# arnauqb/GradABM-JUNE

Measured on AMD Instinct MI355X. Metric: simulation steps/sec, higher is better.
Workload: dtype f32

## Files before the change

### gradabm-june_amd/csrc/gj_compile.hip

```cpp
#include <hip/hip_runtime.h>
#include <hipcub/hipcub.hpp>
#include <stdint.h>

#include <algorithm>

#include "../../include/gradjune_hip.h"

namespace gjc {

constexpr int kThreads = 256;
constexpr int kPad = 8;
constexpr int kChunk = 64;
constexpr int kWideSegments = 6;

static inline int grid_for(int64_t n) { return (int)std::max<int64_t>(1, std::min<int64_t>((n + kThreads - 1) / kThreads, 1 << 18)); }
static inline int grid_for_reduction(int64_t n) { return (int)std::max<int64_t>(1, std::min<int64_t>((n + kThreads - 1) / kThreads, 2048)); }
static inline int64_t align_up(int64_t x) { return (x + 255) & ~(int64_t)255; }
static inline int bits_for(uint64_t n) {
  int b = 0;
  while (b < 64 && (n > ((uint64_t)1 << b))) ++b;
  return std::max(b, 1);
}

__device__ __forceinline__ int upper_bound(const int32_t* a, int n, int64_t x) {
// ... 213 lines not shown
}

__global__ void k_ell_fill(const uint32_t* keys, const uint32_t* order, int64_t E, int64_t n_agents,
                           const int32_t* rowptr, const int64_t* venue, int64_t rows, int32_t ell_k, uint16_t* ell,
                           int32_t* counts) {
  for (int64_t i = (int64_t)blockIdx.x * blockDim.x + threadIdx.x; i < E; i += (int64_t)gridDim.x * blockDim.x) {
    const uint32_t a = keys[i];
    if ((int64_t)a >= n_agents) continue;
    const int col = (int)i - rowptr[a];
    if (col < 0 || col >= ell_k) {
      if (counts) counts[GJ_CC_ERROR] = 5;
      continue;
    }
    ell[((int64_t)(col >> 1) * rows + a) * 2 + (col & 1)] = (uint16_t)venue[order[i]];
  }
}

__global__ void k_explicit_slots(const int32_t* sptr, const int32_t* tile_jpos, int64_t n_tiles, int64_t E, int32_t* slots) {
  for (int64_t i = (int64_t)blockIdx.x * blockDim.x + threadIdx.x; i < E; i += (int64_t)gridDim.x * blockDim.x) {
    int64_t lo = 0, hi = n_tiles + 1;
    while (lo < hi) {
      const int64_t mid = (lo + hi) >> 1;
      if ((int64_t)sptr[mid] > i) {
        hi = mid;
      } else {
        lo = mid + 1;
      }
    }
    const int64_t t = lo - 1;
    slots[i] = tile_jpos[t] + (int32_t)(i - sptr[t]);
// ... 430 lines not shown
  const int64_t need = 2 * gjc::align_up(n1 * 4) + gjc::align_up((int64_t)temp_bytes);
  if (need > workspace_bytes) return GJ_E_RANGE;
  char* base = static_cast<char*>(workspace);
  int32_t* flags = reinterpret_cast<int32_t*>(base);
  int32_t* rows = reinterpret_cast<int32_t*>(base + gjc::align_up(n1 * 4));
  void* temp = base + 2 * gjc::align_up(n1 * 4);
  hipStream_t st = (hipStream_t)stream;
  gjc::k_multi_flags<<<gjc::grid_for(n1), gjc::kThreads, 0, st>>>(desc, n_chunks, wide, flags);
  if (const int rc = gjc::exclusive_scan(temp, temp_bytes, flags, rows, n1, st)) return rc;
  gjc::k_multi_fill<<<gjc::grid_for((int64_t)n_chunks * 64), gjc::kThreads, 0, st>>>(
      out->chunk_ptr, out->tile_sptr, out->tile_jpos, set->n_blocks, set->n_slices, n_chunks, wide, rows, desc, multi_slots,
      counts);
  return (int)hipGetLastError();
}

int gj_compile_runs_pick(const gj_compile_set* set, int32_t* vmin, int32_t* pick, uint8_t* keep, int32_t* win_lo,
                         int32_t* win_n, int32_t* counts, void* stream) {
  if (const int rc = gjc::check_set(set)) return rc;
  if (!vmin || !pick || !counts || !win_lo || !win_n || (set->n_edges > 0 && !keep)) return GJ_E_NULL;
  if (set->n_venues >= gjc::kNoVenue) return GJ_E_RANGE;
  hipStream_t st = (hipStream_t)stream;
  const int64_t A = set->n_agents, E = set->n_edges;
  const int32_t n_own_slices = (int32_t)std::max<int64_t>(1, (A + set->slice_agents - 1) / set->slice_agents);
  GJC_HIP(hipMemsetAsync(counts, 0, GJ_COMPILE_COUNTS * sizeof(int32_t), st));
  if (A > 0) {
    GJC_HIP(hipMemsetD32Async((hipDeviceptr_t)vmin, gjc::kNoVenue, (size_t)A, st));
    GJC_HIP(hipMemsetD32Async((hipDeviceptr_t)pick, gjc::kNoVenue, (size_t)A, st));
  }
  if (E > 0 && A > 0) {
    gjc::k_run_vmin<<<gjc::grid_for(E), gjc::kThreads, 0, st>>>(set->agent, set->venue, E, A, vmin);
// ... 42 lines not shown
```

### gradabm-june_amd/csrc/gj_tiled.h

```cpp
#pragma once
#include <hip/hip_runtime.h>
#include <stdint.h>

#include <type_traits>

#include "../../include/gradjune_hip.h"
#include "gj_device.h"

namespace gj {

constexpr int kTileThreads = 1024;
constexpr int kTileWaves = kTileThreads / kWave;
constexpr int kMaxSliceAgents = 19840;
constexpr int kUnroll = 8;
#ifndef GJ_UNROLL_NARROW
#define GJ_UNROLL_NARROW 16
#endif
constexpr int kUnrollNarrow = GJ_UNROLL_NARROW;
#ifndef GJ_VENUE_UNROLL
#define GJ_VENUE_UNROLL 2
#endif
constexpr int kVenueUnroll = GJ_VENUE_UNROLL;
#ifndef GJ_VENUE_UNROLL_C
#define GJ_VENUE_UNROLL_C GJ_VENUE_UNROLL
// ... 416 lines not shown
      if (T.wide == 2) {
        scatter_explicit<kUnroll>(T, lds_x, s, wave, lane);
      } else if (T.wide) {
        scatter_set<true>(T, lds_x, s, wave, lane);
      } else {
        scatter_set<false>(T, lds_x, s, wave, lane);
      }
    }
  }
}

struct TSetB {
  const int32_t* blk_v0;
  const int32_t* blk_e0;
  const uint16_t* e_lv;
  const uint8_t* e_cls;
  float* val;
  const float* v_pc;
  float* cum;
  int32_t stride;
  int32_t nk;
  float beta[GJ_MAX_NETS_PER_SET];
  int32_t table[GJ_MAX_NETS_PER_SET];
  int32_t age75[GJ_MAX_NETS_PER_SET];
  int32_t leisure;
  int32_t direct;
  uint32_t term_limit;
  int32_t multinet;
  const uint16_t* pv_blk;
  const int32_t* blk_r0;
// ... 61 lines not shown
      : w{raw.x, raw.y, raw.z, raw.w}, c{craw.x, craw.y}, v{xa.x, xa.y, xa.z, xa.w, xb.x, xb.y, xb.z, xb.w} {}
  __device__ __forceinline__ int lv(int q) const { return (w[q >> 1] >> ((q & 1) * 16)) & 0xFFFF; }
  __device__ __forceinline__ float x(int q) const { return v[q]; }
  __device__ __forceinline__ int cls(int q) const { return class_byte(c[q >> 2], q & 3); }
  __device__ __forceinline__ void drop(int q) { w[q >> 1] |= 0xFFFFu << ((q & 1) * 16); }
  __device__ __forceinline__ bool one_venue() const {
    return (w[0] == w[1]) && (w[1] == w[2]) && (w[2] == w[3]) && ((w[0] >> 16) == (w[0] & 0xFFFFu)) && (lv(0) != 0xFFFF);
  }
  __device__ __forceinline__ Group8 weighted(const float* tk) const {
    Group8 g = *this;
#pragma unroll
    for (int q = 0; q < 8; ++q) g.v[q] = tk[cls(q)] * v[q];
    return g;
  }
};

#ifdef GJ_DIAG_STAMPS
constexpr int kDiagVenueSlots = 8192;
__device__ unsigned long long gj_diag_venue[3 * kDiagVenueSlots];
struct VenueStamp {
  unsigned long long t0;
  __device__ VenueStamp() : t0(__builtin_amdgcn_s_memrealtime()) {}
  __device__ ~VenueStamp() {
    if (threadIdx.x == 0 && blockIdx.x < kDiagVenueSlots) {
      gj_diag_venue[3 * blockIdx.x] = t0;
      gj_diag_venue[3 * blockIdx.x + 1] = __builtin_amdgcn_s_memrealtime();
      gj_diag_venue[3 * blockIdx.x + 2] = __builtin_amdgcn_s_getreg((31 << 11) | 20) & 0xF;
    }
  }
};
// ... 8 lines not shown
  int g0, g1;
  fx_t* sums;
  float* cumf;
  int wpad;
  float* tabs;
  float* tabs2;
  uint32_t* vflags;
  int vwords;
  int dummy;
  __device__ __forceinline__ VenueItem(const TSetB& T_, int j, float* lds, int tid_)
      : T(T_), tid(tid_), nk(T_.nk), v0(T_.blk_v0[j]), nv(T_.blk_v0[j + 1] - v0), g0(T_.blk_e0[j] >> 3),
        g1(T_.blk_e0[j + 1] >> 3), sums(reinterpret_cast<fx_t*>(lds)), cumf(lds), wpad(T_.multinet ? class_pad(nk) : 0),
        tabs(lds + 2 * (((size_t)nk * nv + 64 + 1) & ~(size_t)1)), tabs2(tabs + (T_.leisure ? (wpad ? wpad : nk) * 200 : 0)),
        vflags(reinterpret_cast<uint32_t*>(tabs2 + (T_.leisure ? nk * 200 : 0))), vwords((nk * nv + 64 + 31) / 32),
        dummy(nk * nv + (tid_ & 63)) {}
  __device__ __forceinline__ const uint4* lv8() const { return reinterpret_cast<const uint4*>(T.e_lv); }
  __device__ __forceinline__ const uint2* cls8() const { return reinterpret_cast<const uint2*>(T.e_cls); }
  __device__ __forceinline__ float4* val4() const { return reinterpret_cast<float4*>(T.val); }
};

__device__ __forceinline__ void run_sums(const VenueItem& W, const Group8& G, int base_k, fx_t* sums, uint32_t* vflags) {
  const uint32_t kLimit = W.T.term_limit;
  static_assert(kFxVenue == 36, "term_limit is derived from 2^(50 - kFxVenue) (fill_set_b)");
  if (__builtin_expect(max_abs_bits(G.v) > kLimit, 0)) {
    venue_group_slow(sums, vflags, W.vwords, kLimit, base_k, G.lv(0), G.lv(1), G.lv(2), G.lv(3), G.lv(4), G.lv(5),
                     G.lv(6), G.lv(7), G.x(0), G.x(1), G.x(2), G.x(3), G.x(4), G.x(5), G.x(6), G.x(7));
    return;
  }
  fx_t s8 = 0;
#pragma unroll
  for (int q = 0; q < 8; ++q) {
// ... 82 lines not shown
        for (int q = 0; q < 8; ++q) {
          const fx_t f = C.to_fx(x[q]);
          s8 = first[q] ? f : s8 + f;
          if (take[q]) atomicAdd(&sums[base_k + lv[q]], s8);
        }
      }
    }
  }
}

__device__ __forceinline__ void venue_zero(const VenueItem& W, fx_t* sums, uint32_t* vflags) {
  for (int i = W.tid; i < W.nk * W.nv + 64; i += kTileThreads) sums[i] = 0;
  for (int i = W.tid; i < 2 * W.vwords; i += kTileThreads) vflags[i] = 0u;
}

__device__ __forceinline__ void venue_sums_tiled(const VenueItem& W, const float* weights, fx_t* sums, uint32_t* vflags) {
  const TSetB& T = W.T;
  const float wmax = T.multinet ? max_class_weight(weights, 200 * W.wpad, W.tid) : 0.0f;
  const FxConsts<kFxVenue> fxc = FxConsts<kFxVenue>::make();
  auto add_group = [&](const Group8& G) {
    const bool mine = G.one_venue() && (G.lv(0) == __builtin_amdgcn_readfirstlane(G.lv(0)));
    const bool one_venue = __builtin_amdgcn_ballot_w64(mine) == ~0ull;
    if (!T.leisure) {
      if (!(one_venue && one_venue_sum(W, G, G.lv(0), sums))) run_sums(W, G, 0, sums, vflags);
    } else if (T.multinet) {
      multi_sums(W, G, one_venue, weights, wmax, fxc, sums, vflags);
    } else {
      for (int k = 0; k < W.nk; ++k) {
        const Group8 Gk = G.weighted(weights + k * 200);
        if (!(one_venue && one_venue_sum(W, Gk, k * W.nv + G.lv(0), sums))) run_sums(W, Gk, k * W.nv, sums, vflags);
      }
    }
  };
  for (int g = W.g0 + W.tid; g < W.g1; g += kVenueUnroll * kTileThreads) {
    uint4 raw[kVenueUnroll];
    float4 xa[kVenueUnroll], xb[kVenueUnroll];
    uint2 craw[kVenueUnroll];
#pragma unroll
    for (int u = 0; u < kVenueUnroll; ++u) {
      const int gu = min(g + u * kTileThreads, W.g1 - 1);
      raw[u] = W.lv8()[gu];
      xa[u] = load_nt(W.val4() + 2 * gu);
      xb[u] = load_nt(W.val4() + 2 * gu + 1);
      craw[u] = T.leisure ? W.cls8()[gu] : make_uint2(0u, 0u);
    }
#pragma unroll
    for (int u = 0; u < kVenueUnroll; ++u)
      if (g + u * kTileThreads < W.g1) add_group(Group8(raw[u], craw[u], xa[u], xb[u]));
  }
}

__device__ __forceinline__ void venue_sums_runs(const VenueItem& W, int j, fx_t* sums, uint32_t* vflags) {
  const TSetB& T = W.T;
  const int r0 = T.blk_r0[j], r1 = T.blk_r0[j + 1];
  const uint4* pv8 = reinterpret_cast<const uint4*>(T.pv_blk);
  const float4* x4 = reinterpret_cast<const float4*>(T.x);
// ... 57 lines not shown
  for (int k = 0; k < W.nk; ++k) {
    for (int l0 = W.tid; l0 < W.nv; l0 += kCumBatch * kTileThreads) {
      float c[kCumBatch];
#pragma unroll
      for (int u = 0; u < kCumBatch; ++u)
        c[u] = T.cum[(int64_t)(W.v0 + min(l0 + u * kTileThreads, W.nv - 1)) * T.stride + k];
#pragma unroll
      for (int u = 0; u < kCumBatch; ++u) {
        const int lv = l0 + u * kTileThreads;
        if (lv < W.nv) cumf[2 * (k * W.nv + lv)] = c[u];
      }
    }
  }
}

__device__ __forceinline__ void venue_gather(const VenueItem& W, const float* weights, const float* cumf) {
  const TSetB& T = W.T;
  const int nk = W.nk, nv = W.nv;
  for (int g = W.g0 + W.tid; g < W.g1; g += kVenueUnrollC * kTileThreads) {
    uint4 raw[kVenueUnrollC];
    uint2 craw[kVenueUnrollC];
#pragma unroll
    for (int u = 0; u < kVenueUnrollC; ++u) {
      const int gu = min(g + u * kTileThreads, W.g1 - 1);
      raw[u] = W.lv8()[gu];
      craw[u] = T.leisure ? W.cls8()[gu] : make_uint2(0u, 0u);
    }
#pragma unroll
    for (int u = 0; u < kVenueUnrollC; ++u) {
      const int gu = g + u * kTileThreads;
      if (gu >= W.g1) continue;
      const Group8 G(raw[u], craw[u]);
      float r[8];
      if (!T.leisure) {
#pragma unroll
        for (int q = 0; q < 8; ++q) {
          const int lv = G.lv(q);
          const float c = cumf[2 * (lv != 0xFFFF ? lv : 0)];
          r[q] = (lv != 0xFFFF) ? c : 0.0f;
        }
// ... 16 lines not shown

#ifndef GJ_VENUE_WAVES_PER_SIMD
#define GJ_VENUE_WAVES_PER_SIMD 4
#endif
__global__ __launch_bounds__(kTileThreads, GJ_VENUE_WAVES_PER_SIMD) void k_tile_venues(const TileBArgs B) {
  extern __shared__ __align__(16) float lds_s[];
  [[maybe_unused]] const VenueStamp gj_stamp;
  const int set = B.work[2 * blockIdx.x], j = B.work[2 * blockIdx.x + 1];
  const TSetB& T = B.sets[set];
  if (T.nk == 0) return;
  const VenueItem W(T, j, lds_s, threadIdx.x);
  if (T.leisure) fill_class_weights<true, true>(W.tabs, W.tabs2, T, B.tables, B.day_type, B.transpose, W.tid, W.wpad);
  if (B.mode != 2) {
    venue_zero(W, W.sums, W.vflags);
    __syncthreads();
    venue_sums_tiled(W, W.tabs, W.sums, W.vflags);
    if (T.pv_blk) venue_sums_runs(W, j, W.sums, W.vflags);
    __syncthreads();
    venue_cum_write(W, W.sums, W.vflags, W.cumf);
    if (B.mode == 1 || T.direct) return;
  } else {
    if (T.direct) return;
    venue_cum_read(W, W.cumf);
  }
  __syncthreads();
  venue_gather(W, W.tabs2, W.cumf);
}

constexpr int GJ_MAX_PRESUM = 6;
constexpr int64_t kPresumBad = (int64_t)0x8000000000000000ll;
struct TPSet {
  const uint16_t* ell;
  int64_t plane_stride;
  fx_t* partial;
  int32_t planes, V, stride, nk;
  int32_t group_venues;
  int32_t raw, leisure, _pad;
  int32_t table[GJ_MAX_NETS_PER_SET];
  int32_t age75[GJ_MAX_NETS_PER_SET];
};
struct TilePArgs {
// ... 701 lines not shown
```

### gradabm-june_amd/csrc/gradjune_hip.hip

```cpp
#include <hip/hip_runtime.h>
#include <math.h>
#include <stdint.h>
#include <string.h>

#include "../../include/gradjune_hip.h"
#include "gj_device.h"
#include "gj_tiled.h"
#include "gj_agent.h"
#include "gj_location.h"
#include "gj_infector.h"

namespace gj {

struct SetP1 {
  const int32_t* v_rowptr;
  const int32_t* v_agent;
  const float* v_pc;
  float* cum;
  int32_t stride;
  int32_t nk;
  float beta[GJ_MAX_NETS_PER_SET];
  int32_t table[GJ_MAX_NETS_PER_SET];
  int32_t raw;
  int32_t leisure;
// ... 848 lines not shown

static uint32_t venue_term_limit(int32_t max_venue_edges) {
  int e = 14;
  int64_t p2 = 4096;
  while (p2 < (int64_t)max_venue_edges && e > -20) {
    p2 <<= 1;
    --e;
  }
  const float lim = ldexpf(1.0f, e);
  uint32_t bits;
  memcpy(&bits, &lim, sizeof(bits));
  return bits;
}

static int tiled_venues(const gj_plan* plan, const gj_agent_state* st, const gj_step_params* p, const Groups& G, int mode,
                        hipStream_t stream) {
  const gj_tiled* T = plan->tiled;
  if (G.n == 0) return GJ_OK;
  if (T->n_work == 0) return mode == 2 ? GJ_OK : tiled_presum_reduce(plan, p, G, stream);
  TileBArgs B;
  for (int s = 0; s < GJ_MAX_SETS; ++s) B.sets[s] = TSetB{};
  size_t lds = 16;
  for (int g = 0; g < G.n; ++g) {
    const int s = G.set[g];
    const gj_tiled_set& S = T->sets[s];
    const gj_edge_set& E = plan->sets[s];
    TSetB& X = B.sets[s];
    X.blk_v0 = S.blk_v0;
    X.blk_e0 = S.blk_e0;
    X.e_lv = S.e_lv;
    X.e_cls = S.e_cls;
    X.val = S.val;
    X.v_pc = E.v_pcontact;
    X.cum = E.cum;
    X.stride = E.cum_stride;
    X.nk = S.n_blocks > 0 ? G.nk[g] : 0;
    if (uses_presum(plan, s)) X.nk = 0;
    X.direct = S.ell_k != 0;
    const NetGroup C = classify_group(p, G, g);
    X.leisure = C.leisure;
    memcpy(X.beta, C.beta, sizeof(X.beta));
    memcpy(X.table, C.table, sizeof(X.table));
    memcpy(X.age75, C.age75, sizeof(X.age75));
    if (C.leisure && !S.e_cls && E.n_edges > 0) return GJ_E_PLAN;
    if (const int rc = check_group(C)) return rc;
// ... 824 lines not shown
    S.venue = rows[s].a_venue;
    S.n_edges = (int32_t)E.n_edges;
    S.n_venues = (int32_t)E.n_venues;
    S.stride = E.cum_stride;
    S.U = (unsigned long long*)U[s];
  }
  if (plan->n_agents == 0 || A.n_sets == 0) return GJ_OK;
  A.n = plan->n_agents;
  A.flag = new_infected;
  return gj::launch(gj::k_infector_clear, gj::grid_for(A.n, gj::kLocBlocks, gj::kLocLoads * gj::kWave), gj::kThreads, 0,
                    (hipStream_t)stream, A);
}

int gj_step(const gj_plan* plan, const gj_agent_state* state, const gj_step_params* params, const gj_step_io* io,
            void* stream) {
  int rc = gj::check_plan(plan);
  if (rc) return rc;
  gj::Groups G;
  rc = gj::group_networks(plan, params, &G);
  if (rc) return rc;
  rc = gj::check_state(plan, state, params);
  if (rc) return rc;
  rc = gj::do_transmission(plan, state, params, (hipStream_t)stream);
  if (rc) return rc;
  if (plan->tiled) {
    rc = gj::tiled_scatter(plan, state, params, G, (hipStream_t)stream);
    if (rc) return rc;
    rc = gj::tiled_venues(plan, state, params, G, 0, (hipStream_t)stream);
    if (rc) return rc;
    return gj::tiled_agents(plan, state, params, G, io, 1, (hipStream_t)stream);
  }
  rc = gj::do_venue_reduce(plan, state, params, G, (hipStream_t)stream);
  if (rc) return rc;
  return gj::do_agent_gather(plan, state, params, G, io, 1, (hipStream_t)stream);
}

int gj_step_phase(const gj_plan* plan, const gj_agent_state* state, const gj_step_params* params,
                  const gj_step_io* io, int phase, void* stream) {
  int rc = gj::check_plan(plan);
  if (rc) return rc;
  gj::Groups G;
  rc = gj::group_networks(plan, params, &G);
  if (rc) return rc;
  rc = gj::check_state(plan, state, params, phase == 0 || phase == 3);
  if (rc) return rc;
  hipStream_t st = (hipStream_t)stream;
  switch (phase) {
    case 0: return gj::do_transmission(plan, state, params, st);
    case 1: return plan->tiled ? gj::tiled_scatter(plan, state, params, G, st)
                               : gj::do_venue_reduce(plan, state, params, G, st);
    case 2: return plan->tiled ? gj::tiled_venues(plan, state, params, G, 0, st) : GJ_OK;
    case 3: return plan->tiled ? gj::tiled_agents(plan, state, params, G, io, 1, st)
                               : gj::do_agent_gather(plan, state, params, G, io, 1, st);
    case 4: return plan->tiled ? gj::tiled_agents(plan, state, params, G, io, 0, st)
                               : gj::do_agent_gather(plan, state, params, G, io, 0, st);
    case 5: return plan->tiled ? gj::tiled_venues(plan, state, params, G, 1, st) : GJ_OK;
    case 6: return plan->tiled ? gj::tiled_venues(plan, state, params, G, 2, st) : GJ_OK;
    case 7:
    case 8:
      if (!plan->tiled) return gj::do_venue_reduce(plan, state, params, G, st);
      rc = gj::tiled_scatter(plan, state, params, G, st);
      if (rc) return rc;
      return gj::tiled_venues(plan, state, params, G, phase == 7 ? 1 : 0, st);
    default: return GJ_E_RANGE;
  }
}

namespace gj {
__global__ void k_clock_advance(gj_clock* clock, double delta_now) {
  const uint64_t step = clock->step + 1;
  clock->step = step;
  clock->now = (float)(clock->now0 + (double)(int64_t)(step - clock->step0) * delta_now);
}
}

int gj_clock_advance(gj_clock* clock, double delta_now, void* stream) {
  if (!clock) return GJ_E_NULL;
  return gj::launch(gj::k_clock_advance, 1, 1, 0, (hipStream_t)stream, clock, delta_now);
// ... 41 lines not shown
```

### gradabm-june_amd/grad_june_amd/_native.py

```python
from __future__ import annotations

import ctypes as C
import os
from typing import Optional

GJ_ABI_VERSION = 7
GJ_MAX_SETS = 12
GJ_MAX_NETS = 16
GJ_MAX_NETS_PER_SET = 8
GJ_TABLE_SIZE = 400
GJ_ADJ_BETA_BLOCKS = 256
GJ_STREAM_EDGES = 2048
GJ_MAX_GROUPS = 1 << 28
GJ_GROUP_ERR_LABEL, GJ_GROUP_ERR_VALUE = 1, 2
GJ_SEED_CHUNK = 1024
GJ_STAGE_ERR_LABEL, GJ_STAGE_ERR_STAGE = 1, 2
GJ_STAGE_LDS_BINS, GJ_STAGE_ADJ_LDS_BINS = 8192, 2048
GJ_STAGE_LDS_THREADS, GJ_STAGE_LDS_BLOCKS = 1024, 512
GJ_STAGE_GLOBAL_THREADS, GJ_STAGE_GLOBAL_BLOCKS = 256, 2048
GJ_STAGE_LANE_LOADS = 63
GJ_STAGE_MAX_AGENTS = 1 << 40
GJ_LOC_UNIT = 1 << 30
GJ_LOC_ERR_LABEL, GJ_LOC_ERR_VALUE, GJ_LOC_ERR_ROWS = 1, 2, 4
GJ_LOC_MAX_COLS, GJ_LOC_LDS_BINS, GJ_LOC_BLOCKS = 64, 4096, 2048
# ... 126 lines not shown
        ("q_transmission", _vp),
        ("current_stage", _vp),
    ]


class StepIO(C.Structure):
    _fields_ = [
        ("not_infected_probs", _vp),
        ("new_infected", _vp),
        ("exp_noise", _vp),
        ("trans_susc", _vp),
        ("agent_sums", _vp),
    ]


GJ_MAX_STAGES = 16


class SymptomsParams(C.Structure):
    _fields_ = [
        ("n_stages", C.c_int32),
        ("_pad", C.c_int32),
        ("progress", _vp),
        ("next_kind", C.c_int32 * GJ_MAX_STAGES),
        ("next_loc", C.c_float * GJ_MAX_STAGES),
        ("next_scale", C.c_float * GJ_MAX_STAGES),
        ("rec_kind", C.c_int32 * GJ_MAX_STAGES),
        ("rec_loc", C.c_float * GJ_MAX_STAGES),
        ("rec_scale", C.c_float * GJ_MAX_STAGES),
        ("time", C.c_float),
# ... 94 lines not shown
        C.c_int,
        [C.POINTER(Plan), C.POINTER(StepParams), C.POINTER(LocationRows), _vp, _vp, _vp, C.POINTER(_vp), _vp, _vp,
         C.c_int32, _vp, _vp],
    ),
    "gj_infector_gather": (
        C.c_int,
        [C.POINTER(Plan), C.POINTER(StepParams), C.POINTER(LocationRows), _vp, _vp, C.POINTER(_vp), _vp, C.c_int32, _vp,
         _vp, _vp, _vp],
    ),
    "gj_infector_clear": (C.c_int, [C.POINTER(Plan), C.POINTER(LocationRows), _vp, C.POINTER(_vp), _vp]),
    "gj_step": (C.c_int, [C.POINTER(Plan), C.POINTER(AgentState), C.POINTER(StepParams), C.POINTER(StepIO), _vp]),
    "gj_step_phase": (
        C.c_int,
        [C.POINTER(Plan), C.POINTER(AgentState), C.POINTER(StepParams), C.POINTER(StepIO), C.c_int, _vp],
    ),
    "gj_clock_advance": (C.c_int, [_vp, C.c_double, _vp]),
    "gj_symptoms_step_stats": (
        C.c_int,
        [C.c_int64, _vp, _vp, _vp, _vp, _vp, C.POINTER(SymptomsParams), _vp, _vp, _vp, C.c_int32, C.POINTER(C.c_int32),
         C.c_int32, _vp, _vp],
    ),
    "gj_pack_f32": (C.c_int, [C.c_int64, _vp, _vp, _vp, _vp]),
    "gj_unpack_f32": (C.c_int, [C.c_int64, _vp, _vp, _vp, _vp]),
    "gj_event_create": (C.c_int, [C.POINTER(_vp)]),
    "gj_event_record": (C.c_int, [_vp, _vp]),
    "gj_event_elapsed_ms": (C.c_int, [_vp, _vp, C.POINTER(C.c_float)]),
    "gj_event_destroy": (C.c_int, [_vp]),
}

GJ_COMPILE_COUNTS = 16
# ... 16 lines not shown
        ("chunk_ptr", _vp), ("chunk_desc", _vp), ("slots_cap", C.c_int64), ("chunks_cap", C.c_int64),
    ]


_i64p = C.POINTER(C.c_int64)
SYMBOLS.update({
    "gj_compile_capacity": (C.c_int, [C.POINTER(CompileSet), _i64p, _i64p, _i64p]),
    "gj_compile_workspace_bytes": (C.c_int, [C.POINTER(CompileSet), _i64p]),
    "gj_compile_blocks": (C.c_int, [C.POINTER(CompileSet), _vp, C.c_int32, _vp, _vp, C.c_int64, _vp]),
    "gj_compile_tiles": (C.c_int, [C.POINTER(CompileSet), _vp, C.POINTER(CompileOut), _vp, _vp, C.c_int64, _vp]),
    "gj_compile_wide_descriptors": (C.c_int, [C.POINTER(CompileSet), C.POINTER(CompileOut), C.c_int32, _vp, _vp, _vp]),
    "gj_compile_ell_degrees": (C.c_int, [C.POINTER(CompileSet), _vp, _vp, _vp]),
    "gj_compile_explicit_slots": (C.c_int, [C.POINTER(CompileSet), C.POINTER(CompileOut), _vp, _vp]),
    "gj_compile_multi_slots": (C.c_int, [C.POINTER(CompileSet), C.POINTER(CompileOut), C.c_int32, C.c_int32, _vp,
                                          C.c_int32, _vp, _vp, _vp, C.c_int64, _vp]),
    "gj_compile_runs_pick": (C.c_int, [C.POINTER(CompileSet), _vp, _vp, _vp, _vp, _vp, _vp, _vp]),
    "gj_compile_runs_rest": (C.c_int, [C.POINTER(CompileSet), _vp, _vp, _vp, _vp, C.c_int64, _vp, _vp]),
    "gj_compile_runs_index": (C.c_int, [C.POINTER(CompileSet), _vp, _vp, C.c_int32, C.c_int64, _vp, _vp, _vp, _vp, _vp]),
    "gj_compile_ell": (C.c_int, [C.POINTER(CompileSet), C.c_int32, C.c_int64, _vp, _vp, _vp, C.c_int64, _vp, _vp]),
})

_lib: Optional[C.CDLL] = None


class NativeLibraryMissing(RuntimeError):
    pass


def load() -> C.CDLL:
    global _lib
# ... 38 lines not shown
```

### gradabm-june_amd/grad_june_amd/engine.py

```python
from __future__ import annotations

import ctypes as C
import math
from typing import Dict, Optional, Sequence

import torch

from . import _native as N
from .plan import DevicePlan


class AgentBuffers:

    _F32 = ("max_infectiousness", "shape", "rate", "shift", "infection_time", "is_infected",
            "susceptibility", "transmission")

    def __init__(self, plan: DevicePlan, *, max_infectiousness=None, shape=None, rate=None, shift=None,
                 infection_time=None, is_infected=None, susceptibility, transmission, q_transmission=None,
                 current_stage=None):
        n, n_ext = plan.host.n_agents, plan.host.n_ext_agents
        self.tensors = dict(max_infectiousness=max_infectiousness, shape=shape, rate=rate, shift=shift,
                            infection_time=infection_time, is_infected=is_infected,
                            susceptibility=susceptibility, transmission=transmission,
                            q_transmission=q_transmission, current_stage=current_stage)
# ... 31 lines not shown
        self.buf.copy_(torch.from_numpy(host))

    def read(self):
        host = self.buf.cpu().numpy()
        return float(host.view("float32")[0]), int(host[1])

    def advance(self, delta_now: float) -> None:
        N.check(self.lib.gj_clock_advance(self.ptr, float(delta_now), N.current_stream()), "gj_clock_advance")


class InfectionEngine:
    def __init__(self, plan: DevicePlan):
        self.lib = N.load()
        self.plan = plan
        self._q_trans: Optional[torch.Tensor] = None

    def q_transmission_buffer(self) -> torch.Tensor:
        if self._q_trans is None:
            self._q_trans = torch.zeros(self.plan.host.n_ext_agents, dtype=torch.float32, device=self.plan.device)
        return self._q_trans

    def params(self, *, now: float, delta_time: float, day_type: int, active: Sequence[str],
               betas: Dict[str, float], has_quarantine: bool = False, q_threshold: float = math.inf,
               seed: int = 0, step: int = 0, agent_offset: int = 0) -> N.StepParams:
        if len(active) > N.GJ_MAX_NETS:
            raise ValueError(f"at most {N.GJ_MAX_NETS} active networks")
        p = N.StepParams()
        p.now, p.delta_time, p.day_type = float(now), float(delta_time), int(day_type)
        p.has_quarantine = 1 if has_quarantine else 0
        p.q_threshold = float(q_threshold)
# ... 33 lines not shown
        N.check(self.lib.gj_quarantine_transmission(C.byref(self.plan.c), C.byref(bufs.c), C.byref(p),
                                                    N.current_stream()), "gj_quarantine_transmission")

    def venue_reduce(self, bufs: AgentBuffers, p: N.StepParams):
        self._prep(bufs, p)
        N.check(self.lib.gj_venue_reduce(C.byref(self.plan.c), C.byref(bufs.c), C.byref(p),
                                         N.current_stream()), "gj_venue_reduce")

    def agent_gather(self, bufs: AgentBuffers, p: N.StepParams, io: N.StepIO, sample: bool):
        self._prep(bufs, p)
        N.check(self.lib.gj_agent_gather(C.byref(self.plan.c), C.byref(bufs.c), C.byref(p), C.byref(io),
                                         1 if sample else 0, N.current_stream()), "gj_agent_gather")

    def step(self, bufs: AgentBuffers, p: N.StepParams, io: N.StepIO):
        self._prep(bufs, p)
        N.check(self.lib.gj_step(C.byref(self.plan.c), C.byref(bufs.c), C.byref(p), C.byref(io),
                                 N.current_stream()), "gj_step")

    def step_phase(self, bufs: AgentBuffers, p: N.StepParams, io: N.StepIO, phase: int):
        self._prep(bufs, p)
        N.check(self.lib.gj_step_phase(C.byref(self.plan.c), C.byref(bufs.c), C.byref(p), C.byref(io), int(phase),
                                       N.current_stream()), "gj_step_phase")

    def sample_infect(self, not_infected_probs, *, now: float, susceptibility, is_infected, infection_time,
                      exp_noise=None, new_infected=None, seed: int = 0, step: int = 0, agent_offset: int = 0):
        n = not_infected_probs.numel()
        N.check(self.lib.gj_sample_infect(n, N.ptr(not_infected_probs), N.ptr(exp_noise), int(seed), int(step),
                                          int(agent_offset), float(now), N.ptr(new_infected),
                                          N.ptr(susceptibility), N.ptr(is_infected), N.ptr(infection_time),
                                          N.current_stream()), "gj_sample_infect")


class HipTimer:

    def __init__(self):
        self.lib = N.load()
        self.a, self.b = C.c_void_p(), C.c_void_p()
# ... 21 lines not shown
```

### gradabm-june_amd/grad_june_amd/plan.py

```python
from __future__ import annotations

import os

import ctypes as C
from dataclasses import dataclass, field
from typing import Dict, List, Optional, Sequence

import numpy as np
import torch

from . import _native as N
from . import tiling as TL

LONG_CHUNK = 8192
MAX_ROWS_PER_BLOCK = 2048
WORK_NET_COST = 0.15


@dataclass
class HostEdgeSet:
    name: str
    n_venues: int
    n_edges: int
    v_rowptr: Optional[np.ndarray]
# ... 201 lines not shown
                                       chunk_desc=a[p + "tiled/chunk_desc"], desc_wide=bool(wide),
                                       ell=a.get(p + "tiled/ell"), ell_k=ell_k, slot_idx=a.get(p + "tiled/slot_idx"),
                                       multi_slots=a.get(p + "tiled/multi_slots"),
                                       presum=bool(meta[5]) if len(meta) > 5 else False)
            if p + "tiled/runs/meta" in a:
                r = p + "tiled/runs/"
                hs.tiled.n_edges = int(len(a[p + "tiled/a_la"]))
                hs.tiled.runs = TL.RunForm(n_primary=int(a[r + "meta"][0]), keep=None, vmin=a[r + "vmin"],
                                           pv_blk=a[r + "pv_blk"], pv_win=a[r + "pv_win"], blk_r0=a[r + "blk_r0"],
                                           win_lo=a[r + "win_lo"], win_n=a[r + "win_n"], max_window=int(a[r + "meta"][1]))
        sets.append(hs)
    return HostPlan(int(a["meta/n_agents"]), int(a["meta/n_ext_agents"]), sets, a["agent_class"], a["blocks"],
                    a["long_rows"], int(a["meta/n_partial_slots"]), {s.name: i for i, s in enumerate(sets)},
                    layout=str(a["meta/layout"]), n_slices=int(a["meta/n_slices"]),
                    slice_agents=int(a["meta/slice_agents"]), work=a.get("work"))


def agent_class_of(age, sex) -> np.ndarray:
    age = np.asarray(age).astype(np.int64)
    sex = np.asarray(sex).astype(np.int64)
    if age.size and (age.min() < 0 or age.max() > 99 or sex.min() < 0 or sex.max() > 1):
        raise ValueError("age must be in 0..99 and sex in {0,1} (leisure tables are [2,2,100])")
    return (sex * 100 + age).astype(np.uint8)


def compile_plan(n_agents: int, edge_sets: Dict[str, dict], age=None, sex=None,
                 n_ext_agents: Optional[int] = None, block_order: str = "interleave",
                 layout: str = "csr", leisure_sets: Sequence[str] = ("leisure",),
                 sv_max: int = TL.SV_MAX, eb_target: Optional[int] = None, slices=None, tile_pad: int = 1,
                 nets_per_set: Optional[Dict[str, int]] = None, progress=None,
# ... 158 lines not shown
        return None, es
    return rf, dict(es, **rest)


def _finish_runs(rf, t, n_agents: int, slice_agents: int, device):
    if device is not None:
        from .tiling_native import finish_run_form_native

        return finish_run_form_native(rf, t.blk_v0, n_agents, slice_agents, device)
    return TL.finish_run_form(rf, _host(t.blk_v0), n_agents, slice_agents)


class DevicePlan:

    def __init__(self, host: HostPlan, networks: Sequence[NetworkSpec], device, flat_cum_sets: Sequence[str] = (),
                 split_epilogue: bool = False, direct_table_floats: int = 0):
        self.host = host
        self.device = torch.device(device)
        if self.device.type != "cuda":
            raise RuntimeError("grad_june_amd runs the infection path on a HIP device only (no CPU path)")
        self.networks = {n.name: n for n in networks}
        dev = self.device

        def up(a, dtype=None):
            t = a if isinstance(a, torch.Tensor) else torch.from_numpy(np.ascontiguousarray(a))
            if dtype is not None:
                t = t.to(dtype)
            return t.to(dev).contiguous()

        self.table_index: Dict[str, int] = {}
        tabs = []
        for n in networks:
# ... 63 lines not shown
                c.max_block_venues = int(np.diff(_host(ts.blk_v0)).max()) if ts.n_blocks else 0
                c.max_venue_edges = int(min(s.max_venue_edges, 2**31 - 1))
                c.desc_wide = 1 if ts.desc_wide else 0
                if ts.slot_idx is not None and ts.n_edges > 0:
                    t["chunk_desc"] = up(ts.slot_idx)
                    c.desc_wide = 2
                elif ts.multi_slots is not None and len(ts.multi_slots):
                    t["multi_slots"] = up(ts.multi_slots.reshape(-1))
                    c.multi_slots = t["multi_slots"].data_ptr()
                c.blk_v0, c.blk_e0 = t["blk_v0"].data_ptr(), t["blk_e0"].data_ptr()
                c.e_lv, c.a_la = t["e_lv"].data_ptr(), t["a_la"].data_ptr()
                c.e_cls = N.ptr(t.get("e_cls"))
                c.tile_sptr, c.tile_jpos, c.val = t["tile_sptr"].data_ptr(), t["tile_jpos"].data_ptr(), t["val"].data_ptr()
                c.chunk_ptr, c.chunk_desc = t["chunk_ptr"].data_ptr(), N.ptr(t["chunk_desc"])
                c.ell_k, c.ell = int(ts.ell_k), N.ptr(t.get("ell"))
                if ts.runs is not None:
                    rf = ts.runs
                    pad16 = lambda a: torch.cat([a, torch.full((8,), -1, dtype=a.dtype, device=a.device)])
                    t.update(run_pv_blk=pad16(u16(rf.pv_blk)), run_pv_win=pad16(u16(rf.pv_win)), run_blk_r0=up(rf.blk_r0),
                             run_win_lo=up(rf.win_lo), run_win_n=up(rf.win_n))
                    c.run_pv_blk, c.run_pv_win = t["run_pv_blk"].data_ptr(), t["run_pv_win"].data_ptr()
                    c.run_blk_r0, c.run_win_lo, c.run_win_n = (t["run_blk_r0"].data_ptr(), t["run_win_lo"].data_ptr(),
                                                               t["run_win_n"].data_ptr())
                    c.run_max_window = int(rf.max_window)
                    c.run_tiled_edges = int(ts.n_edges)
            self.keep.append(t)
            self.cum.append(cum)
        self.blocks = up(host.blocks.reshape(-1)) if len(host.blocks) else None
        self.long_rows = up(host.long_rows.reshape(-1)) if len(host.long_rows) else None
        self.partial = (torch.zeros(host.n_partial_slots * N.GJ_MAX_NETS_PER_SET, dtype=torch.float32, device=dev)
# ... 87 lines not shown
```

### include/gradjune_hip.h

```cpp
#ifndef GRADJUNE_HIP_H
#define GRADJUNE_HIP_H

#include <stdint.h>

#ifdef __cplusplus
extern "C" {
#endif

#define GJ_ABI_VERSION 7

#define GJ_MAX_SETS 12
#define GJ_MAX_NETS 16
#define GJ_MAX_NETS_PER_SET 8
#define GJ_TABLE_SIZE 400

#define GJ_OK 0
#define GJ_E_NULL (-1)
#define GJ_E_RANGE (-2)
#define GJ_E_PLAN (-3)
#define GJ_E_NODEVICE (-4)

typedef enum gj_mask_kind {
  GJ_MASK_RAW = 0,
  GJ_MASK_Q = 1,
// ... 301 lines not shown
                            const int32_t* cols , double* partial, void* stream);
int gj_adjoint_beta_finish(int32_t n_cols, const double* partial, const float* scale, double* out, void* stream);

int gj_adjoint_symptoms(int64_t n, const uint8_t* agent_class, const float* new_infected,
                        const float* current_stage0, const float* next_stage0, const float* time_to_next_stage0,
                        const gj_symptoms_params* params, const float* progresses, const float* dwell,
                        const float* g_current, const float* g_next, const float* g_time, float* g_current_in,
                        float* g_next_in, float* g_time_in, float* g_new_infected, void* stream);

int gj_step(const gj_plan* plan, const gj_agent_state* state, const gj_step_params* params,
            const gj_step_io* io, void* stream);

int gj_step_phase(const gj_plan* plan, const gj_agent_state* state, const gj_step_params* params,
                  const gj_step_io* io, int phase, void* stream);

int gj_clock_advance(gj_clock* clock, double delta_now, void* stream);

int gj_pack_f32(int64_t n, const int32_t* index, const float* src, float* out, void* stream);
int gj_unpack_f32(int64_t n, const int32_t* index, const float* in, float* dst, void* stream);

#define GJ_COMPILE_COUNTS 16
#define GJ_CC_BLOCKS 0
#define GJ_CC_SLOTS 1
#define GJ_CC_CHUNKS 2
#define GJ_CC_MULTI 3
#define GJ_CC_OWNED_EDGES 4
#define GJ_CC_MAX_DEGREE 5
#define GJ_CC_ERROR 7
#define GJ_CC_RUN_PRIMARY 8
#define GJ_CC_RUN_UNSORTED 9
// ... 29 lines not shown
int gj_compile_workspace_bytes(const gj_compile_set* set, int64_t* bytes);
int gj_compile_blocks(const gj_compile_set* set, int32_t* blk_v0 , int32_t blk_cap,
                      int32_t* counts, void* workspace, int64_t workspace_bytes, void* stream);
int gj_compile_tiles(const gj_compile_set* set, const int32_t* blk_v0, const gj_compile_out* out, int32_t* counts,
                     void* workspace, int64_t workspace_bytes, void* stream);
int gj_compile_wide_descriptors(const gj_compile_set* set, const gj_compile_out* out, int32_t n_chunks,
                                int32_t* desc8 , int32_t* counts, void* stream);
int gj_compile_ell_degrees(const gj_compile_set* set, int32_t* degree, int32_t* counts, void* stream);
int gj_compile_ell(const gj_compile_set* set, int32_t ell_k, int64_t rows, const int32_t* degree, uint16_t* ell,
                   void* workspace, int64_t workspace_bytes, int32_t* counts, void* stream);

int gj_compile_explicit_slots(const gj_compile_set* set, const gj_compile_out* out, int32_t* slots, void* stream);
int gj_compile_multi_slots(const gj_compile_set* set, const gj_compile_out* out, int32_t n_chunks, int32_t wide,
                           int32_t* desc, int32_t n_multi, int32_t* multi_slots, int32_t* counts, void* workspace,
                           int64_t workspace_bytes, void* stream);

int gj_compile_runs_pick(const gj_compile_set* set, int32_t* vmin, int32_t* pick, uint8_t* keep, int32_t* win_lo,
                         int32_t* win_n, int32_t* counts, void* stream);
int gj_compile_runs_rest(const gj_compile_set* set, const uint8_t* keep, int64_t* agent_out, int64_t* venue_out,
                         void* workspace, int64_t workspace_bytes, int32_t* counts, void* stream);
int gj_compile_runs_index(const gj_compile_set* set, const int32_t* vmin, const int32_t* blk_v0, int32_t n_blocks,
                          int64_t rows, const int32_t* win_lo, uint16_t* pv_blk, uint16_t* pv_win, int32_t* blk_r0,
                          void* stream);

int gj_event_create(void** event);
int gj_event_record(void* event, void* stream);
int gj_event_elapsed_ms(void* start, void* stop, float* ms);
int gj_event_destroy(void* event);

#ifdef __cplusplus
// ... 4 lines not shown
```

Baseline: 2115.

## Narrow per-slot local venue ids to uint8 when blocks have at most 255 venues

Builds a uint8 copy of the per-slot local venue id array at plan time for sets whose blocks hold at most 255 venues. The venue sum and gather kernels read it and widen it back to 16-bit in registers with byte-permute instructions. This halves the bytes spent on venue id loads in the memory-bound venue pass. It adds a plan-time kernel, an extra aux struct through the step API, and templated kernel variants, and is on by default through GJ_LV8.

Result: faster. 2137 (median of 6 runs) (+1.1%).

```diff
diff --git a/gradabm-june_amd/csrc/gj_compile.hip b/gradabm-june_amd/csrc/gj_compile.hip
--- a/gradabm-june_amd/csrc/gj_compile.hip
+++ b/gradabm-june_amd/csrc/gj_compile.hip
@@ -251,6 +251,11 @@
     }
     ell[((int64_t)(col >> 1) * rows + a) * 2 + (col & 1)] = (uint16_t)venue[order[i]];
   }
+}
+
+__global__ void k_narrow_venue_ids(const uint16_t* e_lv, int64_t n, uint8_t* e_lv8) {
+  for (int64_t i = (int64_t)blockIdx.x * blockDim.x + threadIdx.x; i < n; i += (int64_t)gridDim.x * blockDim.x)
+    e_lv8[i] = e_lv[i] == 0xFFFF ? (uint8_t)0xFF : (uint8_t)e_lv[i];
 }
 
 __global__ void k_explicit_slots(const int32_t* sptr, const int32_t* tile_jpos, int64_t n_tiles, int64_t E, int32_t* slots) {
@@ -711,6 +716,14 @@
   return (int)hipGetLastError();
 }
 
+int gj_narrow_venue_ids(int64_t n_slots, const uint16_t* e_lv, uint8_t* e_lv8, void* stream) {
+  if (n_slots < 0) return GJ_E_RANGE;
+  if (n_slots == 0) return 0;
+  if (!e_lv || !e_lv8) return GJ_E_NULL;
+  gjc::k_narrow_venue_ids<<<gjc::grid_for(n_slots), gjc::kThreads, 0, (hipStream_t)stream>>>(e_lv, n_slots, e_lv8);
+  return (int)hipGetLastError();
+}
+
 int gj_compile_runs_pick(const gj_compile_set* set, int32_t* vmin, int32_t* pick, uint8_t* keep, int32_t* win_lo,
                          int32_t* win_n, int32_t* counts, void* stream) {
   if (const int rc = gjc::check_set(set)) return rc;
diff --git a/gradabm-june_amd/csrc/gj_tiled.h b/gradabm-june_amd/csrc/gj_tiled.h
--- a/gradabm-june_amd/csrc/gj_tiled.h
+++ b/gradabm-june_amd/csrc/gj_tiled.h
@@ -454,6 +454,7 @@
   const int32_t* blk_v0;
   const int32_t* blk_e0;
   const uint16_t* e_lv;
+  const uint8_t* e_lv8;
   const uint8_t* e_cls;
   float* val;
   const float* v_pc;
@@ -545,6 +546,15 @@
     return g;
   }
 };
+
+__device__ __forceinline__ uint32_t widen_lv_pair(uint32_t four, uint32_t spread) {
+  const uint32_t w = __builtin_amdgcn_perm(0u, four, spread);
+  return __builtin_amdgcn_perm(w, w + 0x7F017F01u, 0x09060804u);
+}
+__device__ __forceinline__ uint4 widen_lv8(uint2 raw) {
+  return make_uint4(widen_lv_pair(raw.x, 0x0c010c00u), widen_lv_pair(raw.x, 0x0c030c02u),
+                    widen_lv_pair(raw.y, 0x0c010c00u), widen_lv_pair(raw.y, 0x0c030c02u));
+}
 
 #ifdef GJ_DIAG_STAMPS
 constexpr int kDiagVenueSlots = 8192;
@@ -583,7 +593,11 @@
         tabs(lds + 2 * (((size_t)nk * nv + 64 + 1) & ~(size_t)1)), tabs2(tabs + (T_.leisure ? (wpad ? wpad : nk) * 200 : 0)),
         vflags(reinterpret_cast<uint32_t*>(tabs2 + (T_.leisure ? nk * 200 : 0))), vwords((nk * nv + 64 + 31) / 32),
         dummy(nk * nv + (tid_ & 63)) {}
-  __device__ __forceinline__ const uint4* lv8() const { return reinterpret_cast<const uint4*>(T.e_lv); }
+  template <bool NARROW>
+  __device__ __forceinline__ uint4 lv8(int g) const {
+    if (NARROW) return widen_lv8(reinterpret_cast<const uint2*>(T.e_lv8)[g]);
+    return reinterpret_cast<const uint4*>(T.e_lv)[g];
+  }
   __device__ __forceinline__ const uint2* cls8() const { return reinterpret_cast<const uint2*>(T.e_cls); }
   __device__ __forceinline__ float4* val4() const { return reinterpret_cast<float4*>(T.val); }
 };
@@ -696,6 +710,7 @@
   for (int i = W.tid; i < 2 * W.vwords; i += kTileThreads) vflags[i] = 0u;
 }
 
+template <bool NARROW>
 __device__ __forceinline__ void venue_sums_tiled(const VenueItem& W, const float* weights, fx_t* sums, uint32_t* vflags) {
   const TSetB& T = W.T;
   const float wmax = T.multinet ? max_class_weight(weights, 200 * W.wpad, W.tid) : 0.0f;
@@ -721,7 +736,7 @@
 #pragma unroll
     for (int u = 0; u < kVenueUnroll; ++u) {
       const int gu = min(g + u * kTileThreads, W.g1 - 1);
-      raw[u] = W.lv8()[gu];
+      raw[u] = W.lv8<NARROW>(gu);
       xa[u] = load_nt(W.val4() + 2 * gu);
       xb[u] = load_nt(W.val4() + 2 * gu + 1);
       craw[u] = T.leisure ? W.cls8()[gu] : make_uint2(0u, 0u);
@@ -809,6 +824,7 @@
   }
 }
 
+template <bool NARROW>
 __device__ __forceinline__ void venue_gather(const VenueItem& W, const float* weights, const float* cumf) {
   const TSetB& T = W.T;
   const int nk = W.nk, nv = W.nv;
@@ -818,7 +834,7 @@
 #pragma unroll
     for (int u = 0; u < kVenueUnrollC; ++u) {
       const int gu = min(g + u * kTileThreads, W.g1 - 1);
-      raw[u] = W.lv8()[gu];
+      raw[u] = W.lv8<NARROW>(gu);
       craw[u] = T.leisure ? W.cls8()[gu] : make_uint2(0u, 0u);
     }
 #pragma unroll
@@ -865,7 +881,11 @@
   if (B.mode != 2) {
     venue_zero(W, W.sums, W.vflags);
     __syncthreads();
-    venue_sums_tiled(W, W.tabs, W.sums, W.vflags);
+    if (T.e_lv8) {
+      venue_sums_tiled<true>(W, W.tabs, W.sums, W.vflags);
+    } else {
+      venue_sums_tiled<false>(W, W.tabs, W.sums, W.vflags);
+    }
     if (T.pv_blk) venue_sums_runs(W, j, W.sums, W.vflags);
     __syncthreads();
     venue_cum_write(W, W.sums, W.vflags, W.cumf);
@@ -875,7 +895,11 @@
     venue_cum_read(W, W.cumf);
   }
   __syncthreads();
-  venue_gather(W, W.tabs2, W.cumf);
+  if (T.e_lv8) {
+    venue_gather<true>(W, W.tabs2, W.cumf);
+  } else {
+    venue_gather<false>(W, W.tabs2, W.cumf);
+  }
 }
 
 constexpr int GJ_MAX_PRESUM = 6;
diff --git a/gradabm-june_amd/csrc/gradjune_hip.hip b/gradabm-june_amd/csrc/gradjune_hip.hip
--- a/gradabm-june_amd/csrc/gradjune_hip.hip
+++ b/gradabm-june_amd/csrc/gradjune_hip.hip
@@ -886,7 +886,7 @@
 }
 
 static int tiled_venues(const gj_plan* plan, const gj_agent_state* st, const gj_step_params* p, const Groups& G, int mode,
-                        hipStream_t stream) {
+                        hipStream_t stream, const gj_aux* aux = nullptr) {
   const gj_tiled* T = plan->tiled;
   if (G.n == 0) return GJ_OK;
   if (T->n_work == 0) return mode == 2 ? GJ_OK : tiled_presum_reduce(plan, p, G, stream);
@@ -901,6 +901,8 @@
     X.blk_v0 = S.blk_v0;
     X.blk_e0 = S.blk_e0;
     X.e_lv = S.e_lv;
+    X.e_lv8 = (aux && !p->transpose) ? aux->e_lv8[s] : nullptr;
+    if (X.e_lv8 && (S.max_block_venues > 255 || (uintptr_t)X.e_lv8 % 8 != 0)) return GJ_E_PLAN;
     X.e_cls = S.e_cls;
     X.val = S.val;
     X.v_pc = E.v_pcontact;
@@ -1755,6 +1757,11 @@
 
 int gj_step(const gj_plan* plan, const gj_agent_state* state, const gj_step_params* params, const gj_step_io* io,
             void* stream) {
+  return gj_step_aux(plan, state, params, io, nullptr, stream);
+}
+
+int gj_step_aux(const gj_plan* plan, const gj_agent_state* state, const gj_step_params* params, const gj_step_io* io,
+                const gj_aux* aux, void* stream) {
   int rc = gj::check_plan(plan);
   if (rc) return rc;
   gj::Groups G;
@@ -1767,7 +1774,7 @@
   if (plan->tiled) {
     rc = gj::tiled_scatter(plan, state, params, G, (hipStream_t)stream);
     if (rc) return rc;
-    rc = gj::tiled_venues(plan, state, params, G, 0, (hipStream_t)stream);
+    rc = gj::tiled_venues(plan, state, params, G, 0, (hipStream_t)stream, aux);
     if (rc) return rc;
     return gj::tiled_agents(plan, state, params, G, io, 1, (hipStream_t)stream);
   }
@@ -1778,6 +1785,11 @@
 
 int gj_step_phase(const gj_plan* plan, const gj_agent_state* state, const gj_step_params* params,
                   const gj_step_io* io, int phase, void* stream) {
+  return gj_step_phase_aux(plan, state, params, io, nullptr, phase, stream);
+}
+
+int gj_step_phase_aux(const gj_plan* plan, const gj_agent_state* state, const gj_step_params* params,
+                      const gj_step_io* io, const gj_aux* aux, int phase, void* stream) {
   int rc = gj::check_plan(plan);
   if (rc) return rc;
   gj::Groups G;
@@ -1790,19 +1802,19 @@
     case 0: return gj::do_transmission(plan, state, params, st);
     case 1: return plan->tiled ? gj::tiled_scatter(plan, state, params, G, st)
                                : gj::do_venue_reduce(plan, state, params, G, st);
-    case 2: return plan->tiled ? gj::tiled_venues(plan, state, params, G, 0, st) : GJ_OK;
+    case 2: return plan->tiled ? gj::tiled_venues(plan, state, params, G, 0, st, aux) : GJ_OK;
     case 3: return plan->tiled ? gj::tiled_agents(plan, state, params, G, io, 1, st)
                                : gj::do_agent_gather(plan, state, params, G, io, 1, st);
     case 4: return plan->tiled ? gj::tiled_agents(plan, state, params, G, io, 0, st)
                                : gj::do_agent_gather(plan, state, params, G, io, 0, st);
-    case 5: return plan->tiled ? gj::tiled_venues(plan, state, params, G, 1, st) : GJ_OK;
-    case 6: return plan->tiled ? gj::tiled_venues(plan, state, params, G, 2, st) : GJ_OK;
+    case 5: return plan->tiled ? gj::tiled_venues(plan, state, params, G, 1, st, aux) : GJ_OK;
+    case 6: return plan->tiled ? gj::tiled_venues(plan, state, params, G, 2, st, aux) : GJ_OK;
     case 7:
     case 8:
       if (!plan->tiled) return gj::do_venue_reduce(plan, state, params, G, st);
       rc = gj::tiled_scatter(plan, state, params, G, st);
       if (rc) return rc;
-      return gj::tiled_venues(plan, state, params, G, phase == 7 ? 1 : 0, st);
+      return gj::tiled_venues(plan, state, params, G, phase == 7 ? 1 : 0, st, aux);
     default: return GJ_E_RANGE;
   }
 }
diff --git a/gradabm-june_amd/grad_june_amd/_native.py b/gradabm-june_amd/grad_june_amd/_native.py
--- a/gradabm-june_amd/grad_june_amd/_native.py
+++ b/gradabm-june_amd/grad_june_amd/_native.py
@@ -164,6 +164,12 @@
     ]
 
 
+class Aux(C.Structure):
+    _fields_ = [
+        ("e_lv8", _vp * GJ_MAX_SETS),
+    ]
+
+
 GJ_MAX_STAGES = 16
 
 
@@ -288,6 +294,12 @@
         C.c_int,
         [C.POINTER(Plan), C.POINTER(AgentState), C.POINTER(StepParams), C.POINTER(StepIO), C.c_int, _vp],
     ),
+    "gj_step_aux": (
+        C.c_int, [C.POINTER(Plan), C.POINTER(AgentState), C.POINTER(StepParams), C.POINTER(StepIO), C.POINTER(Aux), _vp]),
+    "gj_step_phase_aux": (
+        C.c_int,
+        [C.POINTER(Plan), C.POINTER(AgentState), C.POINTER(StepParams), C.POINTER(StepIO), C.POINTER(Aux), C.c_int, _vp],
+    ),
     "gj_clock_advance": (C.c_int, [_vp, C.c_double, _vp]),
     "gj_symptoms_step_stats": (
         C.c_int,
@@ -334,6 +346,7 @@
     "gj_compile_explicit_slots": (C.c_int, [C.POINTER(CompileSet), C.POINTER(CompileOut), _vp, _vp]),
     "gj_compile_multi_slots": (C.c_int, [C.POINTER(CompileSet), C.POINTER(CompileOut), C.c_int32, C.c_int32, _vp,
                                           C.c_int32, _vp, _vp, _vp, C.c_int64, _vp]),
+    "gj_narrow_venue_ids": (C.c_int, [C.c_int64, _vp, _vp, _vp]),
     "gj_compile_runs_pick": (C.c_int, [C.POINTER(CompileSet), _vp, _vp, _vp, _vp, _vp, _vp, _vp]),
     "gj_compile_runs_rest": (C.c_int, [C.POINTER(CompileSet), _vp, _vp, _vp, _vp, C.c_int64, _vp, _vp]),
     "gj_compile_runs_index": (C.c_int, [C.POINTER(CompileSet), _vp, _vp, C.c_int32, C.c_int64, _vp, _vp, _vp, _vp, _vp]),
diff --git a/gradabm-june_amd/grad_june_amd/engine.py b/gradabm-june_amd/grad_june_amd/engine.py
--- a/gradabm-june_amd/grad_june_amd/engine.py
+++ b/gradabm-june_amd/grad_june_amd/engine.py
@@ -69,6 +69,9 @@
         self.lib = N.load()
         self.plan = plan
         self._q_trans: Optional[torch.Tensor] = None
+        self.aux = N.Aux()
+        for i, t in enumerate(plan.lv8):
+            self.aux.e_lv8[i] = N.ptr(t)
 
     def q_transmission_buffer(self) -> torch.Tensor:
         if self._q_trans is None:
@@ -132,13 +135,13 @@
 
     def step(self, bufs: AgentBuffers, p: N.StepParams, io: N.StepIO):
         self._prep(bufs, p)
-        N.check(self.lib.gj_step(C.byref(self.plan.c), C.byref(bufs.c), C.byref(p), C.byref(io),
-                                 N.current_stream()), "gj_step")
+        N.check(self.lib.gj_step_aux(C.byref(self.plan.c), C.byref(bufs.c), C.byref(p), C.byref(io), C.byref(self.aux),
+                                     N.current_stream()), "gj_step")
 
     def step_phase(self, bufs: AgentBuffers, p: N.StepParams, io: N.StepIO, phase: int):
         self._prep(bufs, p)
-        N.check(self.lib.gj_step_phase(C.byref(self.plan.c), C.byref(bufs.c), C.byref(p), C.byref(io), int(phase),
-                                       N.current_stream()), "gj_step_phase")
+        N.check(self.lib.gj_step_phase_aux(C.byref(self.plan.c), C.byref(bufs.c), C.byref(p), C.byref(io),
+                                           C.byref(self.aux), int(phase), N.current_stream()), "gj_step_phase")
 
     def sample_infect(self, not_infected_probs, *, now: float, susceptibility, is_infected, infection_time,
                       exp_noise=None, new_infected=None, seed: int = 0, step: int = 0, agent_offset: int = 0):
diff --git a/gradabm-june_amd/grad_june_amd/plan.py b/gradabm-june_amd/grad_june_amd/plan.py
--- a/gradabm-june_amd/grad_june_amd/plan.py
+++ b/gradabm-june_amd/grad_june_amd/plan.py
@@ -239,6 +239,15 @@
                     a["long_rows"], int(a["meta/n_partial_slots"]), {s.name: i for i, s in enumerate(sets)},
                     layout=str(a["meta/layout"]), n_slices=int(a["meta/n_slices"]),
                     slice_agents=int(a["meta/slice_agents"]), work=a.get("work"))
+
+
+LV8_MAX_BLOCK_VENUES = 255
+
+
+def narrow_venue_ids(e_lv) -> np.ndarray:
+    e = _host(e_lv)
+    e = e.view(np.uint16) if e.dtype == np.int16 else e.astype(np.uint16)
+    return np.where(e == 0xFFFF, 0xFF, e).astype(np.uint8)
 
 
 def agent_class_of(age, sex) -> np.ndarray:
@@ -427,8 +436,11 @@
 class DevicePlan:
 
     def __init__(self, host: HostPlan, networks: Sequence[NetworkSpec], device, flat_cum_sets: Sequence[str] = (),
-                 split_epilogue: bool = False, direct_table_floats: int = 0):
+                 split_epilogue: bool = False, direct_table_floats: int = 0, lv8: Optional[bool] = None):
         self.host = host
+        if lv8 is None:
+            lv8 = os.environ.get("GJ_LV8", "1") != "0"
+        self.lv8: List[Optional[torch.Tensor]] = [None] * len(host.sets)
         self.device = torch.device(device)
         if self.device.type != "cuda":
             raise RuntimeError("grad_june_amd runs the infection path on a HIP device only (no CPU path)")
@@ -522,6 +534,12 @@
                 c.tile_sptr, c.tile_jpos, c.val = t["tile_sptr"].data_ptr(), t["tile_jpos"].data_ptr(), t["val"].data_ptr()
                 c.chunk_ptr, c.chunk_desc = t["chunk_ptr"].data_ptr(), N.ptr(t["chunk_desc"])
                 c.ell_k, c.ell = int(ts.ell_k), N.ptr(t.get("ell"))
+                if lv8 and 0 < c.max_block_venues <= LV8_MAX_BLOCK_VENUES and t["e_lv"].numel():
+                    n_lv = t["e_lv"].numel()
+                    t["e_lv8"] = torch.full((-(-n_lv // 8) * 8,), 0xFF, dtype=torch.uint8, device=dev)
+                    N.check(N.load().gj_narrow_venue_ids(n_lv, t["e_lv"].data_ptr(), t["e_lv8"].data_ptr(),
+                                                         N.current_stream()), "gj_narrow_venue_ids")
+                    self.lv8[i] = t["e_lv8"]
                 if ts.runs is not None:
                     rf = ts.runs
                     pad16 = lambda a: torch.cat([a, torch.full((8,), -1, dtype=a.dtype, device=a.device)])
diff --git a/include/gradjune_hip.h b/include/gradjune_hip.h
--- a/include/gradjune_hip.h
+++ b/include/gradjune_hip.h
@@ -339,6 +339,14 @@
 int gj_step_phase(const gj_plan* plan, const gj_agent_state* state, const gj_step_params* params,
                   const gj_step_io* io, int phase, void* stream);
 
+typedef struct gj_aux {
+  const uint8_t* e_lv8[GJ_MAX_SETS];
+} gj_aux;
+int gj_step_aux(const gj_plan* plan, const gj_agent_state* state, const gj_step_params* params,
+                const gj_step_io* io, const gj_aux* aux, void* stream);
+int gj_step_phase_aux(const gj_plan* plan, const gj_agent_state* state, const gj_step_params* params,
+                      const gj_step_io* io, const gj_aux* aux, int phase, void* stream);
+
 int gj_clock_advance(gj_clock* clock, double delta_now, void* stream);
 
 int gj_pack_f32(int64_t n, const int32_t* index, const float* src, float* out, void* stream);
@@ -398,6 +406,7 @@
 int gj_compile_multi_slots(const gj_compile_set* set, const gj_compile_out* out, int32_t n_chunks, int32_t wide,
                            int32_t* desc, int32_t n_multi, int32_t* multi_slots, int32_t* counts, void* workspace,
                            int64_t workspace_bytes, void* stream);
+int gj_narrow_venue_ids(int64_t n_slots, const uint16_t* e_lv, uint8_t* e_lv8, void* stream);
 
 int gj_compile_runs_pick(const gj_compile_set* set, int32_t* vmin, int32_t* pick, uint8_t* keep, int32_t* win_lo,
                          int32_t* win_n, int32_t* counts, void* stream);
```
